# claussss/ubisoft-laforge-daft-exprt

Hardware: AMD Instinct MI355X
Metric: mel frames/sec (fwd+bwd) (higher is better)
Workload: dtype bf16; 1 GPU; C2: LJ-shaped training step, 48 utterances/GPU, L_max=120, T_max=896, 28180 valid frames/GPU/step; forward + loss (mel L1/L2, adversarial CE, post-mult, energy + pitch consistency) + backward + fused Adam step (global-norm clip, LR schedule) + one-launch weight re-pack, dropout on; parallelism=dp1, launch=1 captured HIP graph(s) per step (one per backward phase) + eager optimiser

## Files before the change

### ubisoft_laforge_daft_exprt_amd/csrc/dx_ffpair.hip

```cpp
#include "dx_common.h"
#include <algorithm>

namespace {

template <int NJ> struct FP {
  static constexpr int NROW = NJ * 16;
  static constexpr int TOK = NROW - 2;
  static constexpr int HR = NROW + 2;
  static constexpr int IMG = 2 * HR * 128;
  static constexpr int XP = (HR * 16 + 511) / 512;
  static constexpr int RP = (HR + 31) / 32;
};
constexpr int FP_TOK = FP<8>::TOK;

struct FFPairArgs {
  const dx_h16* X; int ldx;
  const dx_h16* Wa; const dx_h16* Wb;
  const float* bias_a; const float* bias_b;
  const dx_h16* aux; int ld_aux;
  dx_h16* H; int ldh;
  float* Y; int ldy;
  int B, N, F;
  int accumulate;
  const int* lens; int skip_halo;
  const int* rows_exist;
  const float* ln_res; const float* ln_w; const float* ln_b; const float* film; int ld_film;
  float* ln_y; float* ln_mean; float* ln_rstd;
  unsigned long long seed_pre; unsigned thresh_pre; float inv_keep_pre; const unsigned long long* seed_offset;
  const dx_h16* q_w; const float* q_bias; dx_h16* q_out;
  const float* lnb_z; const float* lnb_mean; const float* lnb_rstd; const float* lnb_w; const float* lnb_b;
  dx_h16* lnb_dg; float* lnb_dw; float* lnb_db;
  const dx_h16* lnb_wt; dx_h16* lnb_datt;
  const float* lnp_dy; const float* lnp_z; const float* lnp_mean; const float* lnp_rstd; const float* lnp_w; const float* lnp_b;
  const float* lnp_film; int lnp_ld_film;
  dx_h16* lnp_dg; float* lnp_dw; float* lnp_db; float* lnp_dfilm; int lnp_ld_dfilm;
  unsigned long long lnp_seed; unsigned lnp_thresh; float lnp_inv_keep;
  unsigned* hmask;
  unsigned long long* stamps;
};

#ifdef DX_FFPAIR_STAMPS
#define FP_STAMP(K) { if (lane == 0 && wq == 0 && a.stamps) a.stamps[((size_t)blockIdx.x * 2 + role) * 16 + (K)] = __builtin_amdgcn_s_memtime(); }
#else
#define FP_STAMP(K) {}
#endif

__device__ __forceinline__ int fp_lds_off(int row, int slot) { return row * 128 + ((slot ^ (row & 7)) << 4); }

__device__ __forceinline__ uint2 fp_pack4(float a, float b, float c, float d) {
  bf16x4 h;
  h[0] = (dx_h16)a; h[1] = (dx_h16)b; h[2] = (dx_h16)c; h[3] = (dx_h16)d;
  return __builtin_bit_cast(uint2, h);
}

__device__ __forceinline__ int fp_opaque(int x) { asm volatile("" : "+v"(x)); return x; }

__device__ __forceinline__ int fp_wave_sum_i(int v) {
#pragma unroll
  for (int off = 32; off > 0; off >>= 1) v += __shfl_xor(v, off, 64);
  return v;
}

typedef short s16x2 __attribute__((ext_vector_type(2)));

#define FP_MMA(W, X, C) C = DX_MFMA_H16(__builtin_bit_cast(bf16x8, W), __builtin_bit_cast(bf16x8, X), C);
// ... 101 lines not shown
        if (a.lnp_w) *reinterpret_cast<f32x4*>(a.lnp_dg + ((size_t)b * a.N + n0 + row) * 128 + q * 8) = f32x4{0.f, 0.f, 0.f, 0.f};
        if (a.lnb_wt) *reinterpret_cast<f32x4*>(a.lnb_datt + ((size_t)b * a.N + n0 + row) * 128 + q * 8) = f32x4{0.f, 0.f, 0.f, 0.f};
      }
    if (a.lnp_w)
      for (int u = tid; u < rows * 32; u += 512) {
        const int row = u >> 5, q = u & 31;
        *reinterpret_cast<f32x4*>(a.Y + ((size_t)b * a.N + n0 + row) * a.ldy + q * 4) = f32x4{0.f, 0.f, 0.f, 0.f};
      }
    if (!a.accumulate)
      for (int u = tid; u < rows * 32; u += 512) {
        const int row = u >> 5, q = u & 31;
        *reinterpret_cast<f32x4*>(a.Y + ((size_t)b * a.N + n0 + row) * a.ldy + q * 4) = f32x4{0.f, 0.f, 0.f, 0.f};
        if (a.ln_w) *reinterpret_cast<f32x4*>(a.ln_y + ((size_t)b * a.N + n0 + row) * 128 + q * 4) = f32x4{0.f, 0.f, 0.f, 0.f};
      }
    if (a.q_w)
      for (int u = tid; u < rows * 48; u += 512) {
        const int row = u / 48, q = u - row * 48;
        *reinterpret_cast<f32x4*>(a.q_out + ((size_t)b * a.N + n0 + row) * 384 + q * 8) = f32x4{0.f, 0.f, 0.f, 0.f};
      }
    return;
  }

  const int NL = a.rows_exist ? a.rows_exist[b] : a.N;
  if (a.lnp_w) {
    const int q = tid & 15;
    const int len_b = a.lens ? a.lens[b] : a.N;
    float wv[8], bv[8], fg[8];
#pragma unroll
    for (int e = 0; e < 8; ++e) {
      wv[e] = a.lnp_w[q * 8 + e]; bv[e] = a.lnp_b[q * 8 + e];
      fg[e] = a.lnp_film ? a.lnp_film[(size_t)b * a.lnp_ld_film + q * 8 + e] : 1.f;
    }
    const unsigned long long seed = a.lnp_seed + (a.seed_offset ? *a.seed_offset : 0ull);
    float gw[8], gb[8], gfg[8], gfb[8];
#pragma unroll
    for (int e = 0; e < 8; ++e) gw[e] = gb[e] = gfg[e] = gfb[e] = 0.f;
    f32x4 dyv[RP][2], zv[RP][2];
    float muv[RP], rsv[RP];
#pragma unroll
    for (int it = 0; it < RP; ++it) {
      const int row = (tid >> 4) + it * 32, n = n0 - 2 + row;
      const bool valid = row < FP_HR && n >= 0 && n < len_b && n < NL;
      const size_t grow = (size_t)b * a.N + n;
#pragma unroll
      for (int hh = 0; hh < 2; ++hh) {
        dyv[it][hh] = valid ? *reinterpret_cast<const f32x4*>(a.lnp_dy + grow * 128 + q * 8 + hh * 4) : f32x4{0.f, 0.f, 0.f, 0.f};
        zv[it][hh] = valid ? *reinterpret_cast<const f32x4*>(a.lnp_z + grow * 128 + q * 8 + hh * 4) : f32x4{0.f, 0.f, 0.f, 0.f};
      }
      muv[it] = valid ? a.lnp_mean[grow] : 0.f;
      rsv[it] = valid ? a.lnp_rstd[grow] : 0.f;
    }
    FP_WLOAD(0, 0) FP_WLOAD(1, 1) FP_WLOAD(2, 2) FP_WLOAD(3, 3)
    if constexpr (RING == 6) { FP_WLOAD(4, 4) FP_WLOAD(5, 5) }
#pragma unroll
    for (int it = 0; it < RP; ++it) {
      const int row = (tid >> 4) + it * 32, n = n0 - 2 + row;
      const bool inb = row < FP_HR && n >= 0 && n < a.N;
      const bool owned = inb && row >= 2 && row < 2 + FP_TOK;
      const bool ownvalid = owned && n < len_b;
      const size_t grow = (size_t)b * a.N + n;
      float dz[8];
      float s1 = 0.f, s2 = 0.f, g[8], xh[8];
#pragma unroll
      for (int e = 0; e < 8; ++e) {
        const float z = zv[it][e >> 2][e & 3];
        float d = dyv[it][e >> 2][e & 3];
        xh[e] = (z - muv[it]) * rsv[it];
        const float ln = xh[e] * wv[e] + bv[e];
        if (ownvalid) { gfg[e] += d * ln; gfb[e] += d; }
        d *= fg[e];
        if (ownvalid) { gw[e] += d * xh[e]; gb[e] += d; }
        g[e] = d * wv[e];
        s1 += g[e]; s2 += g[e] * xh[e];
      }
#pragma unroll
      for (int off = 1; off < 16; off <<= 1) { s1 += __shfl_xor(s1, off, 64); s2 += __shfl_xor(s2, off, 64); }
      s1 *= (1.0f / 128); s2 *= (1.0f / 128);
#pragma unroll
      for (int e = 0; e < 8; ++e) dz[e] = rsv[it] * (g[e] - s1 - xh[e] * s2);
      if (owned) {
        if (dzs && row - 2 < DZ_ROWS) {
          *reinterpret_cast<f32x4*>(dzs + (row - 2) * 128 + q * 8) = f32x4{dz[0], dz[1], dz[2], dz[3]};
          *reinterpret_cast<f32x4*>(dzs + (row - 2) * 128 + q * 8 + 4) = f32x4{dz[4], dz[5], dz[6], dz[7]};
        } else {
          *reinterpret_cast<f32x4*>(a.Y + grow * a.ldy + q * 8) = f32x4{dz[0], dz[1], dz[2], dz[3]};
          *reinterpret_cast<f32x4*>(a.Y + grow * a.ldy + q * 8 + 4) = f32x4{dz[4], dz[5], dz[6], dz[7]};
        }
      }
      if (a.lnp_thresh) {
        float f[8];
        dx_dropout_scale4(seed, (unsigned long long)grow * 128 + q * 8, a.lnp_thresh, a.lnp_inv_keep, f);
        dx_dropout_scale4(seed, (unsigned long long)grow * 128 + q * 8 + 4, a.lnp_thresh, a.lnp_inv_keep, f + 4);
#pragma unroll
        for (int e = 0; e < 8; ++e) dz[e] *= f[e];
      }
      bf16x8 h8;
#pragma unroll
      for (int e = 0; e < 8; ++e) h8[e] = (dx_h16)dz[e];
      const f32x4 hv = __builtin_bit_cast(f32x4, h8);
      if (owned) *reinterpret_cast<f32x4*>(a.lnp_dg + grow * 128 + q * 8) = hv;
      if (row < FP_HR) *reinterpret_cast<f32x4*>(Xs + (q >> 3) * (FP_HR * 128) + fp_lds_off(row, q & 7)) = hv;
    }
#pragma unroll
    for (int e = 0; e < 8; ++e) {
#pragma unroll
      for (int off = 16; off < 64; off <<= 1) {
        gw[e] += __shfl_xor(gw[e], off, 64); gb[e] += __shfl_xor(gb[e], off, 64);
        gfg[e] += __shfl_xor(gfg[e], off, 64); gfb[e] += __shfl_xor(gfb[e], off, 64);
      }
    }
    float* const red = reinterpret_cast<float*>(Hs0);
    if (lane < 16) {
#pragma unroll
      for (int e = 0; e < 8; ++e) {
        red[(wave * 4 + 0) * 128 + q * 8 + e] = gw[e]; red[(wave * 4 + 1) * 128 + q * 8 + e] = gb[e];
        red[(wave * 4 + 2) * 128 + q * 8 + e] = gfg[e]; red[(wave * 4 + 3) * 128 + q * 8 + e] = gfb[e];
      }
    }
    __syncthreads();
    {
      const int quant = tid >> 7, c = tid & 127;
      float t = 0.f;
#pragma unroll
      for (int w8 = 0; w8 < 8; ++w8) t += red[(w8 * 4 + quant) * 128 + c];
      if (t != 0.f) {
        if (quant == 0) atomicAdd(&a.lnp_dw[c], t);
        else if (quant == 1) atomicAdd(&a.lnp_db[c], t);
        else if (a.lnp_dfilm) atomicAdd(&a.lnp_dfilm[(size_t)b * a.lnp_ld_dfilm + (quant == 3 ? 128 : 0) + c], t);
      }
    }
    __syncthreads();
    if (tid < 64) {
      const int img = tid >> 5, rr = NROW + ((tid >> 4) & 1), qq = tid & 15;
      *reinterpret_cast<f32x4*>((img ? Hs1 : Hs0) + (qq >> 3) * (FP_HR * 128) + fp_lds_off(rr, qq & 7)) = f32x4{0.f, 0.f, 0.f, 0.f};
    }
  } else
  {
    f32x4 xr[XP];
#pragma unroll
    for (int it = 0; it < XP; ++it) {
      const int u = tid + it * 512;
      const int row = u >> 4, q = u & 15;
      const int n = n0 - 2 + row;
      f32x4 v = f32x4{0.f, 0.f, 0.f, 0.f};
      if (u < FP_HR * 16 && n >= 0 && n < NL) v = *reinterpret_cast<const f32x4*>(a.X + ((size_t)b * a.N + n) * a.ldx + q * 8);
      xr[it] = v;
    }
    FP_WLOAD(0, 0) FP_WLOAD(1, 1) FP_WLOAD(2, 2) FP_WLOAD(3, 3)
    if constexpr (RING == 6) { FP_WLOAD(4, 4) FP_WLOAD(5, 5) }
    if (tid < 64) {
      const int img = tid >> 5, rr = NROW + ((tid >> 4) & 1), q = tid & 15;
      *reinterpret_cast<f32x4*>((img ? Hs1 : Hs0) + (q >> 3) * (FP_HR * 128) + fp_lds_off(rr, q & 7)) = f32x4{0.f, 0.f, 0.f, 0.f};
    }
#pragma unroll
    for (int it = 0; it < XP; ++it) {
      const int u = tid + it * 512;
      const int row = u >> 4, q = u & 15;
      if (u < FP_HR * 16) *reinterpret_cast<f32x4*>(Xs + (q >> 3) * (FP_HR * 128) + fp_lds_off(row, q & 7)) = xr[it];
    }
  }
  __syncthreads();
  FP_STAMP(2)

  int foff[3][2];
#pragma unroll
  for (int t = 0; t < 3; ++t)
#pragma unroll
    for (int hh = 0; hh < 2; ++hh) foff[t][hh] = fp_lds_off(r + t, hh * 4 + g);
  const int len_cols = min(FP_TOK, a.N - n0);
  const int h_rows = a.H ? len_cols : 0;

#define FP_CO_RD(K, IMGC)                                                                                            \
  {                                                                                                                  \
    const int u_ = fp_opaque(tid) + NROW * 8 + (K) * 256;        \
    const int row_ = u_ >> 4, q_ = u_ & 15;                                                                          \
    cpv = *reinterpret_cast<const f32x4*>((IMGC) + (q_ >> 3) * (FP_HR * 128) + fp_lds_off(min(row_, NROW - 1) + 1, q_ & 7)); \
  }
#define FP_CO_ST(K, F0C)                                                                                             \
  {                                                                                                                  \
    const int u_ = fp_opaque(tid) + NROW * 8 + (K) * 256;                                                            \
    const int row_ = u_ >> 4, q_ = u_ & 15;                                                                          \
    if (row_ < h_rows) *reinterpret_cast<f32x4*>(a.H + ((size_t)b * a.N + n0 + row_) * a.ldh + (F0C) + q_ * 8) = cpv; \
  }
#define FP_COPY_OUT_CONS(IMGC, F0C)                                                                                  \
  {                                                                                                                  \
    f32x4 cv_[NJ / 2];                                                                                               \
    const int t_ = fp_opaque(tid) - 256;                        \
    _Pragma("unroll") for (int k = 0; k < NJ / 2; ++k) {                                                                  \
      const int u_ = t_ + k * 256;                                                                                   \
      cv_[k] = *reinterpret_cast<const f32x4*>((IMGC) + ((u_ & 15) >> 3) * (FP_HR * 128) + fp_lds_off((u_ >> 4) + 1, u_ & 7)); \
    }                                                                                                                \
    _Pragma("unroll") for (int k = 0; k < NJ / 2; ++k) {                                                             \
      const int u_ = t_ + k * 256;                                                                                   \
      const int row_ = u_ >> 4, q_ = u_ & 15;                                                                        \
      if (row_ < h_rows) *reinterpret_cast<f32x4*>(a.H + ((size_t)b * a.N + n0 + row_) * a.ldh + (F0C) + q_ * 8) = cv_[k]; \
    }                                                                                                                \
  }

#define FP_RD8(DST, IMG, S)                                                                                          \
  {                                                                                                                  \
    const unsigned char* const bp_ = (IMG) + (((S) & 3) >> 1) * (FP_HR * 128) + foff[((S) >> 2) % 3][(S) & 1];       \
    _Pragma("unroll") for (int j = 0; j < NJ; ++j) DST[j] = *reinterpret_cast<const float4*>(bp_ + j * 2048);        \
  }
#define FP_STEP(CUR, NXT, IMG, GS0, S, AUXPF, FRESH, CO, IMGC, F0C)                                                  \
  {                                                                                                                  \
    if ((S) + 1 < 12) FP_RD8(NXT, IMG, (S) + 1)                                                                      \
    if ((CO) && (S) < NJ && ((S) & 1) == 0) FP_CO_RD((S) >> 1, IMGC)                                                 \
    __builtin_amdgcn_sched_barrier(0);                                                                               \
    const f32x4 w0 = wr[(S) % RING][0], w1 = wr[(S) % RING][1];                                                      \
    if ((FRESH) && (S) == 0) {                                   \
      _Pragma("unroll") for (int j = 0; j < NJ; ++j) { acc[0][j] = bv0; FP_MMA(w0, CUR[j], acc[0][j]) }              \
      _Pragma("unroll") for (int j = 0; j < NJ; ++j) { acc[1][j] = bv1; FP_MMA(w1, CUR[j], acc[1][j]) }              \
    } else {                                                                                                         \
      _Pragma("unroll") for (int j = 0; j < NJ; ++j) { FP_MMA(w0, CUR[j], acc[0][j]) }                               \
      _Pragma("unroll") for (int j = 0; j < NJ; ++j) { FP_MMA(w1, CUR[j], acc[1][j]) }                               \
    }                                                                                                                \
    FP_WLOAD((S) % RING, (GS0) + (S) + RING)                                                                         \
    if ((CO) && (S) < NJ && ((S) & 1) == 1) FP_CO_ST((S) >> 1, F0C)                                                  \
    if ((S) == 8) { AUXPF }                                                                                          \
    __builtin_amdgcn_sched_barrier(0);                                                                               \
  }
#define FP_SLICE_STEPS(IMG, GS0, AUXPF, FR, CO, IMGC, F0C)                                                           \
  {                                                                                                                  \
    float4 xa[NJ], xb[NJ];                                                                                           \
    f32x4 cpv;                                                                                                       \
    FP_RD8(xa, IMG, 0)                                                                                               \
    FP_STEP(xa, xb, IMG, GS0, 0, AUXPF, FR, CO, IMGC, F0C) FP_STEP(xb, xa, IMG, GS0, 1, AUXPF, FR, CO, IMGC, F0C)    \
    FP_STEP(xa, xb, IMG, GS0, 2, AUXPF, FR, CO, IMGC, F0C) FP_STEP(xb, xa, IMG, GS0, 3, AUXPF, FR, CO, IMGC, F0C)    \
    FP_STEP(xa, xb, IMG, GS0, 4, AUXPF, FR, CO, IMGC, F0C) FP_STEP(xb, xa, IMG, GS0, 5, AUXPF, FR, CO, IMGC, F0C)    \
    FP_STEP(xa, xb, IMG, GS0, 6, AUXPF, FR, CO, IMGC, F0C) FP_STEP(xb, xa, IMG, GS0, 7, AUXPF, FR, CO, IMGC, F0C)    \
    FP_STEP(xa, xb, IMG, GS0, 8, AUXPF, FR, CO, IMGC, F0C) FP_STEP(xb, xa, IMG, GS0, 9, AUXPF, FR, CO, IMGC, F0C)    \
    FP_STEP(xa, xb, IMG, GS0, 10, AUXPF, FR, CO, IMGC, F0C) FP_STEP(xb, xa, IMG, GS0, 11, AUXPF, FR, CO, IMGC, F0C)  \
  }

  unsigned char* const stage = smem;
  if (role == 0) {
    f32x4 acc[2][NJ];
    const bool edge = n0 == 0 || n0 + FP_TOK >= NL;
    const int tile_lin = b * tiles_n + n0 / FP_TOK;
#define FP_PRODUCE(F_, COFLAG)                                                                                       \
    {                                                                                                                \
      const int f0 = (F_) << 7;                                                                                      \
                                   \
      const f32x4 bv0 = a.bias_a ? *reinterpret_cast<const f32x4*>(a.bias_a + f0 + 32 * wq + 4 * g) : f32x4{0.f, 0.f, 0.f, 0.f};      \
      const f32x4 bv1 = a.bias_a ? *reinterpret_cast<const f32x4*>(a.bias_a + f0 + 32 * wq + 16 + 4 * g) : f32x4{0.f, 0.f, 0.f, 0.f}; \
      bf16x4 av[2][MASK ? 1 : NJ];                                                                                   \
      unsigned mw[2] = {0u, 0u};                                                                                     \
      FP_SLICE_STEPS(Xs, (F_) * 12,                                                                                  \
        if constexpr (AUX) {                                                                                         \
          if constexpr (MASK) {                                                                                      \
            const unsigned* mp_ = a.hmask + ((((size_t)tile_lin * nslices + (f0 >> 7)) * 4 + wq) * 2) * 64 + fp_opaque(lane); \
            mw[0] = mp_[0]; mw[1] = mp_[64];                                                                         \
          } else {                                                                                                   \
          const int r2_ = fp_opaque(r);                                                                              \
          const int g2_ = fp_opaque(g);                                                                              \
          _Pragma("unroll") for (int i = 0; i < 2; ++i)                                                              \
            _Pragma("unroll") for (int j = 0; j < NJ; ++j) {                                                         \
              const int n = min(max(n0 - 1 + 16 * j + r2_, 0), a.N - 1);                                             \
              av[i][j] = *reinterpret_cast<const bf16x4*>(a.aux + ((size_t)b * a.N + n) * a.ld_aux + f0 + 32 * wq + 16 * i + 4 * g2_); \
            }                                                                                                        \
          }                                                                                                          \
        }, true, COFLAG, ((((F_) - 1) & 1) ? Hs1 : Hs0), ((F_) - 1) * 128)                                           \
      unsigned char* const out = ((F_) & 1) ? Hs1 : Hs0;                                                             \
      const int r_ = fp_opaque(r);                                                                                   \
      const int g_ = fp_opaque(g);                                                                                   \
      _Pragma("unroll") for (int i = 0; i < 2; ++i) {                                                                \
        const int c = 32 * wq + 16 * i + 4 * g_;                                                                     \
        unsigned char* const orow = out + (c >> 6) * (FP_HR * 128) + fp_lds_off(r_, (c & 63) >> 3) + ((g_ & 1) << 3); \
        unsigned sw_ = 0u;                                                  \
        const unsigned mwi_ = mw[i];                                                                                 \
        _Pragma("unroll") for (int j = 0; j < NJ; ++j) {                                                             \
          f32x4 v = acc[i][j];                                                                                       \
          if constexpr (AUX) {                                                                                       \
            if constexpr (MASK) {                                                                                    \
               \
              _Pragma("unroll") for (int e = 0; e < 4; ++e) {                                                        \
                const float ve_ = v[e];                                                                              \
                const unsigned ke_ = __float_as_uint(ve_) & (unsigned)__builtin_amdgcn_sbfe((int)mwi_, NJ * 4 - 1 - (j * 4 + e), 1); \
                v[e] = __uint_as_float(ke_);                                                                         \
              }                                                                                                      \
            } else {                                                                                                 \
              _Pragma("unroll") for (int e = 0; e < 4; ++e) if (!((float)av[i][j][e] > 0.f)) v[e] = 0.f;             \
            }                                                                                                        \
          }                                                                                                          \
          if (edge) { const int n = n0 - 1 + 16 * j + r_; if (n < 0 || n >= NL) v = f32x4{0.f, 0.f, 0.f, 0.f}; }    \
          if constexpr (RELU) {                                                                                      \
             \
            if (a.hmask) {                                                                                           \
              _Pragma("unroll") for (int e = 0; e < 4; ++e) {                                                        \
                const float ve_ = v[e];                                                                              \
                sw_ = __builtin_amdgcn_alignbit(sw_, __float_as_uint(ve_) - 1u, 31);                                 \
              }                                                                                                      \
            }                                                                                                        \
          }                                                                                                          \
          uint2 pk = fp_pack4(v[0], v[1], v[2], v[3]);                                                               \
          if constexpr (RELU) {                                                                                      \
             \
            pk.x = __builtin_bit_cast(unsigned, __builtin_elementwise_max(__builtin_bit_cast(s16x2, pk.x), s16x2{0, 0})); \
            pk.y = __builtin_bit_cast(unsigned, __builtin_elementwise_max(__builtin_bit_cast(s16x2, pk.y), s16x2{0, 0})); \
          }                                                                                                          \
          *reinterpret_cast<uint2*>(orow + j * 2048) = pk;                                                           \
        }                                                                                                            \
        if constexpr (RELU) {                                        \
          if (a.hmask) a.hmask[((((size_t)tile_lin * nslices + (f0 >> 7)) * 4 + wq) * 2 + i) * 64 + fp_opaque(lane)] = ~sw_; \
        }                                                                                                            \
      }                                                                                                              \
    }
    FP_PRODUCE(0, false)
    __syncthreads();
    FP_STAMP(3)
    for (int it = 1; it < nslices; ++it) {
      if (it == 4) FP_STAMP(12)
      FP_PRODUCE(it, true)
      if (it == 4) FP_STAMP(14)
      __syncthreads();
      FP_STAMP(3 + it)
    }
    {
      const unsigned char* const imgc = ((nslices - 1) & 1) ? Hs1 : Hs0;
      f32x4 cpv;
#pragma unroll
      for (int k = 0; k < NJ / 2; ++k) { FP_CO_RD(k, imgc) FP_CO_ST(k, (nslices - 1) << 7) }
    }
    __syncthreads();
    FP_STAMP(3 + nslices)
#undef FP_PRODUCE
  } else {
    f32x4 acc[2][NJ];
    const f32x4 bv0 = f32x4{0.f, 0.f, 0.f, 0.f}, bv1 = bv0;
#pragma unroll
    for (int i = 0; i < 2; ++i)
#pragma unroll
      for (int j = 0; j < NJ; ++j) acc[i][j] = f32x4{0.f, 0.f, 0.f, 0.f};
    __syncthreads();
    FP_STAMP(3)
    for (int it = 1; it <= nslices; ++it) {
      if (it == 4) FP_STAMP(12)
      const int f = it - 1;
      const unsigned char* const img = (f & 1) ? Hs1 : Hs0;
      FP_COPY_OUT_CONS(img, f << 7)
      FP_SLICE_STEPS(img, f * 12, , false, false, img, 0)
      if (it == 4) FP_STAMP(13)
      __syncthreads();
      FP_STAMP(3 + it)
    }
#pragma unroll
    for (int i = 0; i < 2; ++i) {
      const int co = 32 * wq + 16 * i + 4 * g;
      const f32x4 bv = a.bias_b ? *reinterpret_cast<const f32x4*>(a.bias_b + co) : f32x4{0.f, 0.f, 0.f, 0.f};
#pragma unroll
      for (int j = 0; j < NJ; ++j) {
        const int q = 16 * j + r;
        *reinterpret_cast<f32x4*>(stage + q * 512 + (((co >> 2) ^ (q & 15)) << 4)) = acc[i][j] + bv;
      }
    }
  }
#undef FP_SLICE_STEPS
#undef FP_STEP
#undef FP_RD8
#undef FP_COPY_OUT_CONS
#undef FP_CO_RD
#undef FP_CO_ST

  __syncthreads();
  if (a.ln_w) {
    const int s = tid & 31;
    const f32x4 wv = *reinterpret_cast<const f32x4*>(a.ln_w + s * 4), bv = *reinterpret_cast<const f32x4*>(a.ln_b + s * 4);
    f32x4 fg = f32x4{1.f, 1.f, 1.f, 1.f}, fb = f32x4{0.f, 0.f, 0.f, 0.f};
    if (a.film) {
      fg = *reinterpret_cast<const f32x4*>(a.film + (size_t)b * a.ld_film + s * 4);
      fb = *reinterpret_cast<const f32x4*>(a.film + (size_t)b * a.ld_film + 128 + s * 4);
    }
    const int len_b = a.lens ? a.lens[b] : a.N;
    const unsigned long long seed = a.seed_pre + (a.seed_offset ? *a.seed_offset : 0ull);
    bf16x8 qa[3][4];
    if (a.q_w) {
#pragma unroll
      for (int i = 0; i < 3; ++i)
#pragma unroll
        for (int ks = 0; ks < 4; ++ks) qa[i][ks] = *reinterpret_cast<const bf16x8*>(a.q_w + (size_t)((wave * 3 + i) * 4 + ks) * 512 + lane * 8);
    }
    f32x4 resv[NJ];
#pragma unroll
    for (int k = 0; k < NJ; ++k) {
      const int row = (tid >> 5) + k * 16, n = n0 + row;
      resv[k] = (row < len_cols && n < len_b) ? *reinterpret_cast<const f32x4*>(a.ln_res + ((size_t)b * a.N + n) * 128 + s * 4) : f32x4{0.f, 0.f, 0.f, 0.f};
    }
#pragma unroll
    for (int k = 0; k < NJ; ++k) {
      const int row = (tid >> 5) + k * 16, n = n0 + row;
      const bool inb = row < len_cols, valid = inb && n < len_b;
      const size_t grow = (size_t)b * a.N + n;
      f32x4 z = f32x4{0.f, 0.f, 0.f, 0.f};
      if (valid) {
        z = *reinterpret_cast<const f32x4*>(stage + row * 512 + ((s ^ (row & 15)) << 4));
        if (a.thresh_pre) {
          float f[4];
          dx_dropout_scale4(seed, (unsigned long long)grow * 128 + s * 4, a.thresh_pre, a.inv_keep_pre, f);
          z[0] *= f[0]; z[1] *= f[1]; z[2] *= f[2]; z[3] *= f[3];
        }
        z += resv[k];
      }
      if (inb) *reinterpret_cast<f32x4*>(a.Y + grow * a.ldy + s * 4) = z;
      float sum = (z[0] + z[1]) + (z[2] + z[3]);
#pragma unroll
      for (int off = 1; off < 32; off <<= 1) sum += __shfl_xor(sum, off, 64);
      const float mu = sum * (1.0f / 128);
      const f32x4 d = z - mu;
      float q = (d[0] * d[0] + d[1] * d[1]) + (d[2] * d[2] + d[3] * d[3]);
#pragma unroll
// ... 21 lines not shown
        bf16x8 xb[4];
#pragma unroll
        for (int ks = 0; ks < 4; ++ks) xb[ks] = *reinterpret_cast<const bf16x8*>(stage + row * 512 + (((ks * 4 + g) ^ (row & 15)) << 4));
        f32x4 acc[3];
#pragma unroll
        for (int i = 0; i < 3; ++i) acc[i] = qb[i];
#pragma unroll
        for (int ks = 0; ks < 4; ++ks)
#pragma unroll
          for (int i = 0; i < 3; ++i) acc[i] = DX_MFMA_H16(qa[i][ks], xb[ks], acc[i]);
        if (row < len_cols) {
          dx_h16* const orow = a.q_out + ((size_t)b * a.N + n0 + row) * 384 + wave * 48 + g * 4;
#pragma unroll
          for (int i = 0; i < 3; ++i) {
            bf16x4 o4;
            o4[0] = (dx_h16)acc[i][0]; o4[1] = (dx_h16)acc[i][1]; o4[2] = (dx_h16)acc[i][2]; o4[3] = (dx_h16)acc[i][3];
            *reinterpret_cast<bf16x4*>(orow + i * 16) = o4;
          }
        }
      }
    }
  } else if (a.lnb_w) {
    const int s = tid & 31;
    const f32x4 wv = *reinterpret_cast<const f32x4*>(a.lnb_w + s * 4), bv = *reinterpret_cast<const f32x4*>(a.lnb_b + s * 4);
    (void)bv;
    const int len_b = a.lens ? a.lens[b] : a.N;
    const unsigned long long seed = a.seed_pre + (a.seed_offset ? *a.seed_offset : 0ull);
    f32x4 oldv[NJ], zv[NJ];
    float muv[NJ], rsv[NJ];
#pragma unroll
    for (int k = 0; k < NJ; ++k) {
      const int row = (tid >> 5) + k * 16, n = n0 + row;
      const bool valid = row < len_cols && n < len_b;
      const size_t grow = (size_t)b * a.N + n;
      if (dzs && row < DZ_ROWS) oldv[k] = valid ? *reinterpret_cast<const f32x4*>(dzs + row * 128 + s * 4) : f32x4{0.f, 0.f, 0.f, 0.f};
      else oldv[k] = valid ? *reinterpret_cast<const f32x4*>(a.Y + grow * a.ldy + s * 4) : f32x4{0.f, 0.f, 0.f, 0.f};
      zv[k] = valid ? *reinterpret_cast<const f32x4*>(a.lnb_z + grow * 128 + s * 4) : f32x4{0.f, 0.f, 0.f, 0.f};
      muv[k] = valid ? a.lnb_mean[grow] : 0.f;
      rsv[k] = valid ? a.lnb_rstd[grow] : 0.f;
    }
    f32x4 gw = f32x4{0.f, 0.f, 0.f, 0.f}, gb = gw;
#pragma unroll
    for (int k = 0; k < NJ; ++k) {
      const int row = (tid >> 5) + k * 16, n = n0 + row;
      const bool inb = row < len_cols, valid = inb && n < len_b;
      const size_t grow = (size_t)b * a.N + n;
      f32x4 d = f32x4{0.f, 0.f, 0.f, 0.f};
      if (valid) d = *reinterpret_cast<const f32x4*>(stage + row * 512 + ((s ^ (row & 15)) << 4)) + oldv[k];
      const f32x4 xh = (zv[k] - muv[k]) * rsv[k];
      gw += d * xh; gb += d;
      const f32x4 g = d * wv;
      float s1 = (g[0] + g[1]) + (g[2] + g[3]);
      const f32x4 gx = g * xh;
      float s2 = (gx[0] + gx[1]) + (gx[2] + gx[3]);
#pragma unroll
      for (int off = 1; off < 32; off <<= 1) { s1 += __shfl_xor(s1, off, 64); s2 += __shfl_xor(s2, off, 64); }
      s1 *= (1.0f / 128); s2 *= (1.0f / 128);
      f32x4 dz = (g - s1 - xh * s2) * rsv[k];
      if (!inb) continue;
      *reinterpret_cast<f32x4*>(a.Y + grow * a.ldy + s * 4) = dz;
      if (a.thresh_pre) {
        float f[4];
        dx_dropout_scale4(seed, (unsigned long long)grow * 128 + s * 4, a.thresh_pre, a.inv_keep_pre, f);
        dz[0] *= f[0]; dz[1] *= f[1]; dz[2] *= f[2]; dz[3] *= f[3];
      }
      bf16x4 h4;
      h4[0] = (dx_h16)dz[0]; h4[1] = (dx_h16)dz[1]; h4[2] = (dx_h16)dz[2]; h4[3] = (dx_h16)dz[3];
      *reinterpret_cast<bf16x4*>(a.lnb_dg + grow * 128 + s * 4) = h4;
      if (a.lnb_wt) *reinterpret_cast<bf16x4*>(stage + row * 512 + (((s >> 1) ^ (row & 15)) << 4) + ((s & 1) << 3)) = h4;
    }
    if (a.lnb_wt) {
#pragma unroll
      for (int k = 0; k < NJ; ++k) {
        const int row = (tid >> 5) + k * 16;
        if (row >= len_cols) *reinterpret_cast<uint2*>(stage + row * 512 + (((s >> 1) ^ (row & 15)) << 4) + ((s & 1) << 3)) = make_uint2(0u, 0u);
      }
    }
    float* const red = reinterpret_cast<float*>(smem + NROW * 512);
    *reinterpret_cast<f32x4*>(red + (tid >> 5) * 128 + s * 4) = gw;
    *reinterpret_cast<f32x4*>(red + 2048 + (tid >> 5) * 128 + s * 4) = gb;
    __syncthreads();
    if (tid < 256) {
      const float* src = red + (tid >> 7) * 2048 + (tid & 127);
      float t = 0.f;
#pragma unroll
      for (int q = 0; q < 16; ++q) t += src[q * 128];
      if (t != 0.f) atomicAdd((tid >> 7) ? &a.lnb_db[tid & 127] : &a.lnb_dw[tid & 127], t);
    }
    if (a.lnb_wt) {
      constexpr int CB = NJ;
      const int rb = wave % NJ, cb0 = (wave / NJ) * CB;
      const int row = rb * 16 + r;
      bf16x8 xb[4];
#pragma unroll
      for (int ks = 0; ks < 4; ++ks) xb[ks] = *reinterpret_cast<const bf16x8*>(stage + row * 512 + (((ks * 4 + g) ^ (row & 15)) << 4));
      f32x4 acc[CB];
#pragma unroll
      for (int i = 0; i < CB; ++i) acc[i] = f32x4{0.f, 0.f, 0.f, 0.f};
#pragma unroll
      for (int ks = 0; ks < 4; ++ks) {
        bf16x8 wa[CB];
#pragma unroll
        for (int i = 0; i < CB; ++i) wa[i] = *reinterpret_cast<const bf16x8*>(a.lnb_wt + (size_t)((cb0 + i) * 4 + ks) * 512 + lane * 8);
#pragma unroll
        for (int i = 0; i < CB; ++i) acc[i] = DX_MFMA_H16(wa[i], xb[ks], acc[i]);
      }
      if (row < len_cols) {
        dx_h16* const orow = a.lnb_datt + ((size_t)b * a.N + n0 + row) * 128 + cb0 * 16 + g * 4;
#pragma unroll
        for (int i = 0; i < CB; ++i) {
          bf16x4 o4;
          o4[0] = (dx_h16)acc[i][0]; o4[1] = (dx_h16)acc[i][1]; o4[2] = (dx_h16)acc[i][2]; o4[3] = (dx_h16)acc[i][3];
          *reinterpret_cast<bf16x4*>(orow + i * 16) = o4;
        }
      }
    }
  } else {
    f32x4 old[NJ];
    if (a.accumulate) {
#pragma unroll
      for (int k = 0; k < NJ; ++k) {
        const int u = tid + k * 512;
        const int row = min(u >> 5, len_cols - 1), s = u & 31;
        old[k] = *reinterpret_cast<const f32x4*>(a.Y + ((size_t)b * a.N + n0 + row) * a.ldy + s * 4);
      }
    }
#pragma unroll
    for (int k = 0; k < NJ; ++k) {
      const int u = tid + k * 512;
// ... 167 lines not shown
```

Before: 4.804 million valid mel frames/s.

## Split LN-backward prologue across roles and prefetch epilogue operands before final sync

For the aux NJ=8 fused FF-pair kernel, the LN-backward prologue rows are split. Role 0 finishes its part early and starts the first producer slice in two halves, while role 1 processes the remaining halo rows and does the parameter-gradient reduction, removing the block-wide barrier before the GEMM. Epilogue operands (LN weights, film, residual/z rows, mean/rstd, q_w fragments, lnb_wt weights) are now fetched into registers before the last barrier so their latency overlaps compute. This raises register pressure and adds complex role-dependent synchronisation, which risks spills, occupancy loss or barrier mismatch.

```diff
diff --git a/ubisoft_laforge_daft_exprt_amd/csrc/dx_ffpair.hip b/ubisoft_laforge_daft_exprt_amd/csrc/dx_ffpair.hip
--- a/ubisoft_laforge_daft_exprt_amd/csrc/dx_ffpair.hip
+++ b/ubisoft_laforge_daft_exprt_amd/csrc/dx_ffpair.hip
@@ -40,7 +40,7 @@
 };
 
 #ifdef DX_FFPAIR_STAMPS
-#define FP_STAMP(K) { if (lane == 0 && wq == 0 && a.stamps) a.stamps[((size_t)blockIdx.x * 2 + role) * 16 + (K)] = __builtin_amdgcn_s_memtime(); }
+#define FP_STAMP(K) { if (lane == 0 && wq == 0 && a.stamps) a.stamps[((size_t)blockIdx.x * 2 + role) * 24 + (K)] = __builtin_amdgcn_s_memtime(); }
 #else
 #define FP_STAMP(K) {}
 #endif
@@ -188,6 +188,10 @@
   }
 
   const int NL = a.rows_exist ? a.rows_exist[b] : a.N;
+  constexpr bool SPLIT = AUX && NJ == 8;
+  constexpr int PA = SPLIT ? 3 : RP;
+  constexpr int PB = SPLIT ? (FP_HR - PA * 32 + 15) / 16 : 0;
+  const bool split0 = SPLIT && a.lnp_w != nullptr;
   if (a.lnp_w) {
     const int q = tid & 15;
     const int len_b = a.lens ? a.lens[b] : a.N;
@@ -201,26 +205,20 @@
     float gw[8], gb[8], gfg[8], gfb[8];
 #pragma unroll
     for (int e = 0; e < 8; ++e) gw[e] = gb[e] = gfg[e] = gfb[e] = 0.f;
-    f32x4 dyv[RP][2], zv[RP][2];
-    float muv[RP], rsv[RP];
-#pragma unroll
-    for (int it = 0; it < RP; ++it) {
-      const int row = (tid >> 4) + it * 32, n = n0 - 2 + row;
+    auto row_load = [&](int row, f32x4 (&dy)[2], f32x4 (&z)[2], float& mu, float& rs) {
+      const int n = n0 - 2 + row;
       const bool valid = row < FP_HR && n >= 0 && n < len_b && n < NL;
       const size_t grow = (size_t)b * a.N + n;
 #pragma unroll
       for (int hh = 0; hh < 2; ++hh) {
-        dyv[it][hh] = valid ? *reinterpret_cast<const f32x4*>(a.lnp_dy + grow * 128 + q * 8 + hh * 4) : f32x4{0.f, 0.f, 0.f, 0.f};
-        zv[it][hh] = valid ? *reinterpret_cast<const f32x4*>(a.lnp_z + grow * 128 + q * 8 + hh * 4) : f32x4{0.f, 0.f, 0.f, 0.f};
-      }
-      muv[it] = valid ? a.lnp_mean[grow] : 0.f;
-      rsv[it] = valid ? a.lnp_rstd[grow] : 0.f;
-    }
-    FP_WLOAD(0, 0) FP_WLOAD(1, 1) FP_WLOAD(2, 2) FP_WLOAD(3, 3)
-    if constexpr (RING == 6) { FP_WLOAD(4, 4) FP_WLOAD(5, 5) }
-#pragma unroll
-    for (int it = 0; it < RP; ++it) {
-      const int row = (tid >> 4) + it * 32, n = n0 - 2 + row;
+        dy[hh] = valid ? *reinterpret_cast<const f32x4*>(a.lnp_dy + grow * 128 + q * 8 + hh * 4) : f32x4{0.f, 0.f, 0.f, 0.f};
+        z[hh] = valid ? *reinterpret_cast<const f32x4*>(a.lnp_z + grow * 128 + q * 8 + hh * 4) : f32x4{0.f, 0.f, 0.f, 0.f};
+      }
+      mu = valid ? a.lnp_mean[grow] : 0.f;
+      rs = valid ? a.lnp_rstd[grow] : 0.f;
+    };
+    auto row_pass = [&](int row, const f32x4 (&dy)[2], const f32x4 (&zz)[2], float mu, float rs) {
+      const int n = n0 - 2 + row;
       const bool inb = row < FP_HR && n >= 0 && n < a.N;
       const bool owned = inb && row >= 2 && row < 2 + FP_TOK;
       const bool ownvalid = owned && n < len_b;
@@ -229,9 +227,9 @@
       float s1 = 0.f, s2 = 0.f, g[8], xh[8];
 #pragma unroll
       for (int e = 0; e < 8; ++e) {
-        const float z = zv[it][e >> 2][e & 3];
-        float d = dyv[it][e >> 2][e & 3];
-        xh[e] = (z - muv[it]) * rsv[it];
+        const float z = zz[e >> 2][e & 3];
+        float d = dy[e >> 2][e & 3];
+        xh[e] = (z - mu) * rs;
         const float ln = xh[e] * wv[e] + bv[e];
         if (ownvalid) { gfg[e] += d * ln; gfb[e] += d; }
         d *= fg[e];
@@ -243,7 +241,7 @@
       for (int off = 1; off < 16; off <<= 1) { s1 += __shfl_xor(s1, off, 64); s2 += __shfl_xor(s2, off, 64); }
       s1 *= (1.0f / 128); s2 *= (1.0f / 128);
 #pragma unroll
-      for (int e = 0; e < 8; ++e) dz[e] = rsv[it] * (g[e] - s1 - xh[e] * s2);
+      for (int e = 0; e < 8; ++e) dz[e] = rs * (g[e] - s1 - xh[e] * s2);
       if (owned) {
         if (dzs && row - 2 < DZ_ROWS) {
           *reinterpret_cast<f32x4*>(dzs + (row - 2) * 128 + q * 8) = f32x4{dz[0], dz[1], dz[2], dz[3]};
@@ -266,39 +264,102 @@
       const f32x4 hv = __builtin_bit_cast(f32x4, h8);
       if (owned) *reinterpret_cast<f32x4*>(a.lnp_dg + grow * 128 + q * 8) = hv;
       if (row < FP_HR) *reinterpret_cast<f32x4*>(Xs + (q >> 3) * (FP_HR * 128) + fp_lds_off(row, q & 7)) = hv;
-    }
-#pragma unroll
-    for (int e = 0; e < 8; ++e) {
-#pragma unroll
-      for (int off = 16; off < 64; off <<= 1) {
-        gw[e] += __shfl_xor(gw[e], off, 64); gb[e] += __shfl_xor(gb[e], off, 64);
-        gfg[e] += __shfl_xor(gfg[e], off, 64); gfb[e] += __shfl_xor(gfb[e], off, 64);
-      }
-    }
-    float* const red = reinterpret_cast<float*>(Hs0);
-    if (lane < 16) {
+    };
+    auto wave_fold = [&]() {
 #pragma unroll
       for (int e = 0; e < 8; ++e) {
-        red[(wave * 4 + 0) * 128 + q * 8 + e] = gw[e]; red[(wave * 4 + 1) * 128 + q * 8 + e] = gb[e];
-        red[(wave * 4 + 2) * 128 + q * 8 + e] = gfg[e]; red[(wave * 4 + 3) * 128 + q * 8 + e] = gfb[e];
-      }
-    }
-    __syncthreads();
-    {
-      const int quant = tid >> 7, c = tid & 127;
-      float t = 0.f;
-#pragma unroll
-      for (int w8 = 0; w8 < 8; ++w8) t += red[(w8 * 4 + quant) * 128 + c];
+#pragma unroll
+        for (int off = 16; off < 64; off <<= 1) {
+          gw[e] += __shfl_xor(gw[e], off, 64); gb[e] += __shfl_xor(gb[e], off, 64);
+          gfg[e] += __shfl_xor(gfg[e], off, 64); gfb[e] += __shfl_xor(gfb[e], off, 64);
+        }
+      }
+    };
+    auto red_atomic = [&](int quant, int c, float t) {
       if (t != 0.f) {
         if (quant == 0) atomicAdd(&a.lnp_dw[c], t);
         else if (quant == 1) atomicAdd(&a.lnp_db[c], t);
         else if (a.lnp_dfilm) atomicAdd(&a.lnp_dfilm[(size_t)b * a.lnp_ld_dfilm + (quant == 3 ? 128 : 0) + c], t);
       }
-    }
-    __syncthreads();
-    if (tid < 64) {
-      const int img = tid >> 5, rr = NROW + ((tid >> 4) & 1), qq = tid & 15;
-      *reinterpret_cast<f32x4*>((img ? Hs1 : Hs0) + (qq >> 3) * (FP_HR * 128) + fp_lds_off(rr, qq & 7)) = f32x4{0.f, 0.f, 0.f, 0.f};
+    };
+    {
+      f32x4 dyv[PA][2], zv[PA][2];
+      float muv[PA], rsv[PA];
+#pragma unroll
+      for (int it = 0; it < PA; ++it) row_load((tid >> 4) + it * 32, dyv[it], zv[it], muv[it], rsv[it]);
+      FP_WLOAD(0, 0) FP_WLOAD(1, 1) FP_WLOAD(2, 2) FP_WLOAD(3, 3)
+      if constexpr (RING == 6) { FP_WLOAD(4, 4) FP_WLOAD(5, 5) }
+#pragma unroll
+      for (int it = 0; it < PA; ++it) row_pass((tid >> 4) + it * 32, dyv[it], zv[it], muv[it], rsv[it]);
+    }
+    if constexpr (SPLIT) {
+      if (tid < 64) {
+        const int img = tid >> 5, rr = NROW + ((tid >> 4) & 1), qq = tid & 15;
+        *reinterpret_cast<f32x4*>((img ? Hs1 : Hs0) + (qq >> 3) * (FP_HR * 128) + fp_lds_off(rr, qq & 7)) = f32x4{0.f, 0.f, 0.f, 0.f};
+      }
+      float* const red = reinterpret_cast<float*>(Hs1);
+      if (role == 0) {
+        wave_fold();
+        if (lane < 16) {
+#pragma unroll
+          for (int e = 0; e < 8; ++e) {
+            red[(wq * 4 + 0) * 128 + q * 8 + e] = gw[e]; red[(wq * 4 + 1) * 128 + q * 8 + e] = gb[e];
+            red[(wq * 4 + 2) * 128 + q * 8 + e] = gfg[e]; red[(wq * 4 + 3) * 128 + q * 8 + e] = gfb[e];
+          }
+        }
+        __syncthreads();
+      } else {
+        f32x4 dyv[PB][2], zv[PB][2];
+        float muv[PB], rsv[PB];
+        const int row0 = PA * 32 + ((tid - 256) >> 4);
+#pragma unroll
+        for (int it = 0; it < PB; ++it) row_load(row0 + it * 16, dyv[it], zv[it], muv[it], rsv[it]);
+        __syncthreads();
+        FP_STAMP(2)
+#pragma unroll
+        for (int it = 0; it < PB; ++it) row_pass(row0 + it * 16, dyv[it], zv[it], muv[it], rsv[it]);
+        wave_fold();
+        if (lane < 16) {
+#pragma unroll
+          for (int e = 0; e < 8; ++e) {
+            red[(wq * 4 + 0) * 128 + q * 8 + e] += gw[e]; red[(wq * 4 + 1) * 128 + q * 8 + e] += gb[e];
+            red[(wq * 4 + 2) * 128 + q * 8 + e] += gfg[e]; red[(wq * 4 + 3) * 128 + q * 8 + e] += gfb[e];
+          }
+        }
+        __syncthreads();
+        FP_STAMP(16)
+#pragma unroll
+        for (int hh = 0; hh < 2; ++hh) {
+          const int u = tid - 256 + hh * 256, quant = u >> 7, c = u & 127;
+          float t = 0.f;
+#pragma unroll
+          for (int w4 = 0; w4 < 4; ++w4) t += red[(w4 * 4 + quant) * 128 + c];
+          red_atomic(quant, c, t);
+        }
+      }
+    } else {
+      wave_fold();
+      float* const red = reinterpret_cast<float*>(Hs0);
+      if (lane < 16) {
+#pragma unroll
+        for (int e = 0; e < 8; ++e) {
+          red[(wave * 4 + 0) * 128 + q * 8 + e] = gw[e]; red[(wave * 4 + 1) * 128 + q * 8 + e] = gb[e];
+          red[(wave * 4 + 2) * 128 + q * 8 + e] = gfg[e]; red[(wave * 4 + 3) * 128 + q * 8 + e] = gfb[e];
+        }
+      }
+      __syncthreads();
+      {
+        const int quant = tid >> 7, c = tid & 127;
+        float t = 0.f;
+#pragma unroll
+        for (int w8 = 0; w8 < 8; ++w8) t += red[(w8 * 4 + quant) * 128 + c];
+        red_atomic(quant, c, t);
+      }
+      __syncthreads();
+      if (tid < 64) {
+        const int img = tid >> 5, rr = NROW + ((tid >> 4) & 1), qq = tid & 15;
+        *reinterpret_cast<f32x4*>((img ? Hs1 : Hs0) + (qq >> 3) * (FP_HR * 128) + fp_lds_off(rr, qq & 7)) = f32x4{0.f, 0.f, 0.f, 0.f};
+      }
     }
   } else
   {
@@ -325,8 +386,8 @@
       if (u < FP_HR * 16) *reinterpret_cast<f32x4*>(Xs + (q >> 3) * (FP_HR * 128) + fp_lds_off(row, q & 7)) = xr[it];
     }
   }
-  __syncthreads();
-  FP_STAMP(2)
+  if (!split0) __syncthreads();
+  if (!(split0 && role == 1)) FP_STAMP(2)
 
   int foff[3][2];
 #pragma unroll
@@ -363,48 +424,105 @@
     }                                                                                                                \
   }
 
-#define FP_RD8(DST, IMG, S)                                                                                          \
+#define FP_RD8(DST, IMG, S, JLO, JHI)                                                                                \
   {                                                                                                                  \
     const unsigned char* const bp_ = (IMG) + (((S) & 3) >> 1) * (FP_HR * 128) + foff[((S) >> 2) % 3][(S) & 1];       \
-    _Pragma("unroll") for (int j = 0; j < NJ; ++j) DST[j] = *reinterpret_cast<const float4*>(bp_ + j * 2048);        \
-  }
-#define FP_STEP(CUR, NXT, IMG, GS0, S, AUXPF, FRESH, CO, IMGC, F0C)                                                  \
+    _Pragma("unroll") for (int j = (JLO); j < (JHI); ++j) DST[j] = *reinterpret_cast<const float4*>(bp_ + j * 2048); \
+  }
+#define FP_STEP(CUR, NXT, IMG, GS0, S, AUXPF, FRESH, CO, IMGC, F0C, JLO, JHI, WRAP)                                                \
   {                                                                                                                  \
-    if ((S) + 1 < 12) FP_RD8(NXT, IMG, (S) + 1)                                                                      \
+    if ((S) + 1 < 12) FP_RD8(NXT, IMG, (S) + 1, JLO, JHI)                                                            \
     if ((CO) && (S) < NJ && ((S) & 1) == 0) FP_CO_RD((S) >> 1, IMGC)                                                 \
     __builtin_amdgcn_sched_barrier(0);                                                                               \
     const f32x4 w0 = wr[(S) % RING][0], w1 = wr[(S) % RING][1];                                                      \
     if ((FRESH) && (S) == 0) {                                   \
-      _Pragma("unroll") for (int j = 0; j < NJ; ++j) { acc[0][j] = bv0; FP_MMA(w0, CUR[j], acc[0][j]) }              \
-      _Pragma("unroll") for (int j = 0; j < NJ; ++j) { acc[1][j] = bv1; FP_MMA(w1, CUR[j], acc[1][j]) }              \
+      _Pragma("unroll") for (int j = (JLO); j < (JHI); ++j) { acc[0][j] = bv0; FP_MMA(w0, CUR[j], acc[0][j]) }       \
+      _Pragma("unroll") for (int j = (JLO); j < (JHI); ++j) { acc[1][j] = bv1; FP_MMA(w1, CUR[j], acc[1][j]) }       \
     } else {                                                                                                         \
-      _Pragma("unroll") for (int j = 0; j < NJ; ++j) { FP_MMA(w0, CUR[j], acc[0][j]) }                               \
-      _Pragma("unroll") for (int j = 0; j < NJ; ++j) { FP_MMA(w1, CUR[j], acc[1][j]) }                               \
+      _Pragma("unroll") for (int j = (JLO); j < (JHI); ++j) { FP_MMA(w0, CUR[j], acc[0][j]) }                        \
+      _Pragma("unroll") for (int j = (JLO); j < (JHI); ++j) { FP_MMA(w1, CUR[j], acc[1][j]) }                        \
     }                                                                                                                \
-    FP_WLOAD((S) % RING, (GS0) + (S) + RING)                                                                         \
+     \
+    FP_WLOAD((S) % RING, (GS0) + ((WRAP) ? ((S) + RING) % 12 : (S) + RING))                                          \
     if ((CO) && (S) < NJ && ((S) & 1) == 1) FP_CO_ST((S) >> 1, F0C)                                                  \
     if ((S) == 8) { AUXPF }                                                                                          \
     __builtin_amdgcn_sched_barrier(0);                                                                               \
   }
-#define FP_SLICE_STEPS(IMG, GS0, AUXPF, FR, CO, IMGC, F0C)                                                           \
+#define FP_SLICE_STEPS(IMG, GS0, AUXPF, FR, CO, IMGC, F0C, JLO, JHI, WRAP)                                          \
   {                                                                                                                  \
     float4 xa[NJ], xb[NJ];                                                                                           \
     f32x4 cpv;                                                                                                       \
-    FP_RD8(xa, IMG, 0)                                                                                               \
-    FP_STEP(xa, xb, IMG, GS0, 0, AUXPF, FR, CO, IMGC, F0C) FP_STEP(xb, xa, IMG, GS0, 1, AUXPF, FR, CO, IMGC, F0C)    \
-    FP_STEP(xa, xb, IMG, GS0, 2, AUXPF, FR, CO, IMGC, F0C) FP_STEP(xb, xa, IMG, GS0, 3, AUXPF, FR, CO, IMGC, F0C)    \
-    FP_STEP(xa, xb, IMG, GS0, 4, AUXPF, FR, CO, IMGC, F0C) FP_STEP(xb, xa, IMG, GS0, 5, AUXPF, FR, CO, IMGC, F0C)    \
-    FP_STEP(xa, xb, IMG, GS0, 6, AUXPF, FR, CO, IMGC, F0C) FP_STEP(xb, xa, IMG, GS0, 7, AUXPF, FR, CO, IMGC, F0C)    \
-    FP_STEP(xa, xb, IMG, GS0, 8, AUXPF, FR, CO, IMGC, F0C) FP_STEP(xb, xa, IMG, GS0, 9, AUXPF, FR, CO, IMGC, F0C)    \
-    FP_STEP(xa, xb, IMG, GS0, 10, AUXPF, FR, CO, IMGC, F0C) FP_STEP(xb, xa, IMG, GS0, 11, AUXPF, FR, CO, IMGC, F0C)  \
+    FP_RD8(xa, IMG, 0, JLO, JHI)                                                                                     \
+    FP_STEP(xa, xb, IMG, GS0, 0, AUXPF, FR, CO, IMGC, F0C, JLO, JHI, WRAP) FP_STEP(xb, xa, IMG, GS0, 1, AUXPF, FR, CO, IMGC, F0C, JLO, JHI, WRAP)   \
+    FP_STEP(xa, xb, IMG, GS0, 2, AUXPF, FR, CO, IMGC, F0C, JLO, JHI, WRAP) FP_STEP(xb, xa, IMG, GS0, 3, AUXPF, FR, CO, IMGC, F0C, JLO, JHI, WRAP)   \
+    FP_STEP(xa, xb, IMG, GS0, 4, AUXPF, FR, CO, IMGC, F0C, JLO, JHI, WRAP) FP_STEP(xb, xa, IMG, GS0, 5, AUXPF, FR, CO, IMGC, F0C, JLO, JHI, WRAP)   \
+    FP_STEP(xa, xb, IMG, GS0, 6, AUXPF, FR, CO, IMGC, F0C, JLO, JHI, WRAP) FP_STEP(xb, xa, IMG, GS0, 7, AUXPF, FR, CO, IMGC, F0C, JLO, JHI, WRAP)   \
+    FP_STEP(xa, xb, IMG, GS0, 8, AUXPF, FR, CO, IMGC, F0C, JLO, JHI, WRAP) FP_STEP(xb, xa, IMG, GS0, 9, AUXPF, FR, CO, IMGC, F0C, JLO, JHI, WRAP)   \
+    FP_STEP(xa, xb, IMG, GS0, 10, AUXPF, FR, CO, IMGC, F0C, JLO, JHI, WRAP) FP_STEP(xb, xa, IMG, GS0, 11, AUXPF, FR, CO, IMGC, F0C, JLO, JHI, WRAP) \
   }
 
   unsigned char* const stage = smem;
+  f32x4 ev[NJ], e_wv, e_bv, e_fg, e_fb;
+  float emu[NJ], ers[NJ];
+  bf16x8 e_qa[3][4];
+#define FP_EPI_FETCH                                                                                                 \
+  {                                                                                                                  \
+    const int s_ = fp_opaque(tid) & 31, t5_ = fp_opaque(tid) >> 5;                                                   \
+    if constexpr (AUX) {                                                                                             \
+      if (a.lnb_w) {                                                                                                 \
+        const int len_b_ = a.lens ? a.lens[b] : a.N;                                                                 \
+        e_wv = *reinterpret_cast<const f32x4*>(a.lnb_w + s_ * 4);                                                    \
+        _Pragma("unroll") for (int k = 0; k < NJ; ++k) {                                                             \
+          const int row = t5_ + k * 16, n = n0 + row;                                                                \
+          const bool valid = row < len_cols && n < len_b_;                                                           \
+          const size_t grow = (size_t)b * a.N + n;                                                                   \
+          ev[k] = valid ? *reinterpret_cast<const f32x4*>(a.lnb_z + grow * 128 + s_ * 4) : f32x4{0.f, 0.f, 0.f, 0.f}; \
+          emu[k] = valid ? a.lnb_mean[grow] : 0.f;                                                                   \
+          ers[k] = valid ? a.lnb_rstd[grow] : 0.f;                                                                   \
+        }                                                                                                            \
+      }                                                                                                              \
+    } else {                                                                                                         \
+      if (a.ln_w) {                                                                                                  \
+        const int len_b_ = a.lens ? a.lens[b] : a.N;                                                                 \
+        e_wv = *reinterpret_cast<const f32x4*>(a.ln_w + s_ * 4); e_bv = *reinterpret_cast<const f32x4*>(a.ln_b + s_ * 4); \
+        e_fg = f32x4{1.f, 1.f, 1.f, 1.f}; e_fb = f32x4{0.f, 0.f, 0.f, 0.f};                                          \
+        if (a.film) {                                                                                                \
+          e_fg = *reinterpret_cast<const f32x4*>(a.film + (size_t)b * a.ld_film + s_ * 4);                           \
+          e_fb = *reinterpret_cast<const f32x4*>(a.film + (size_t)b * a.ld_film + 128 + s_ * 4);                     \
+        }                                                                                                            \
+        if (a.q_w) {                                                    \
+          _Pragma("unroll") for (int i = 0; i < 3; ++i)                                                              \
+            _Pragma("unroll") for (int ks = 0; ks < 4; ++ks)                                                         \
+              e_qa[i][ks] = *reinterpret_cast<const bf16x8*>(a.q_w + (size_t)((wave * 3 + i) * 4 + ks) * 512 + fp_opaque(lane) * 8); \
+        }                                                                                                            \
+        _Pragma("unroll") for (int k = 0; k < NJ; ++k) {                                                             \
+          const int row = t5_ + k * 16, n = n0 + row;                                                                \
+          ev[k] = (row < len_cols && n < len_b_) ? *reinterpret_cast<const f32x4*>(a.ln_res + ((size_t)b * a.N + n) * 128 + s_ * 4) \
+                                                 : f32x4{0.f, 0.f, 0.f, 0.f};                                        \
+        }                                                                                                            \
+      }                                                                                                              \
+    }                                                                                                                \
+  }
   if (role == 0) {
     f32x4 acc[2][NJ];
     const bool edge = n0 == 0 || n0 + FP_TOK >= NL;
     const int tile_lin = b * tiles_n + n0 / FP_TOK;
-#define FP_PRODUCE(F_, COFLAG)                                                                                       \
+#define FP_AUX_PREFETCH                                                                                              \
+    if constexpr (AUX) {                                                                                             \
+      if constexpr (MASK) {                                                                                          \
+        const unsigned* mp_ = a.hmask + ((((size_t)tile_lin * nslices + (f0 >> 7)) * 4 + wq) * 2) * 64 + fp_opaque(lane);\
+        mw[0] = mp_[0]; mw[1] = mp_[64];                                                                             \
+      } else {                                                                                                       \
+      const int r2_ = fp_opaque(r);                                                                                  \
+      const int g2_ = fp_opaque(g);                                                                                  \
+      _Pragma("unroll") for (int i = 0; i < 2; ++i)                                                                  \
+        _Pragma("unroll") for (int j = 0; j < NJ; ++j) {                                                             \
+          const int n = min(max(n0 - 1 + 16 * j + r2_, 0), a.N - 1);                                                 \
+          av[i][j] = *reinterpret_cast<const bf16x4*>(a.aux + ((size_t)b * a.N + n) * a.ld_aux + f0 + 32 * wq + 16 * i + 4 * g2_);\
+        }                                                                                                            \
+      }                                                                                                              \
+    }
+#define FP_PRODUCE(F_, COFLAG, SPLIT0)                                                                                       \
     {                                                                                                                \
       const int f0 = (F_) << 7;                                                                                      \
                                    \
@@ -412,21 +530,16 @@
       const f32x4 bv1 = a.bias_a ? *reinterpret_cast<const f32x4*>(a.bias_a + f0 + 32 * wq + 16 + 4 * g) : f32x4{0.f, 0.f, 0.f, 0.f}; \
       bf16x4 av[2][MASK ? 1 : NJ];                                                                                   \
       unsigned mw[2] = {0u, 0u};                                                                                     \
-      FP_SLICE_STEPS(Xs, (F_) * 12,                                                                                  \
-        if constexpr (AUX) {                                                                                         \
-          if constexpr (MASK) {                                                                                      \
-            const unsigned* mp_ = a.hmask + ((((size_t)tile_lin * nslices + (f0 >> 7)) * 4 + wq) * 2) * 64 + fp_opaque(lane); \
-            mw[0] = mp_[0]; mw[1] = mp_[64];                                                                         \
-          } else {                                                                                                   \
-          const int r2_ = fp_opaque(r);                                                                              \
-          const int g2_ = fp_opaque(g);                                                                              \
-          _Pragma("unroll") for (int i = 0; i < 2; ++i)                                                              \
-            _Pragma("unroll") for (int j = 0; j < NJ; ++j) {                                                         \
-              const int n = min(max(n0 - 1 + 16 * j + r2_, 0), a.N - 1);                                             \
-              av[i][j] = *reinterpret_cast<const bf16x4*>(a.aux + ((size_t)b * a.N + n) * a.ld_aux + f0 + 32 * wq + 16 * i + 4 * g2_); \
-            }                                                                                                        \
-          }                                                                                                          \
-        }, true, COFLAG, ((((F_) - 1) & 1) ? Hs1 : Hs0), ((F_) - 1) * 128)                                           \
+      if (SPLIT0) {                                                                                                  \
+         \
+                    \
+        FP_SLICE_STEPS(Xs, 0, , true, false, Hs0, 0, 0, NJ / 2, true)                                                \
+        __syncthreads();                                                                                             \
+        FP_STAMP(16)                                                                                                 \
+        FP_SLICE_STEPS(Xs, 0, FP_AUX_PREFETCH, true, false, Hs0, 0, NJ / 2, NJ, false)                               \
+      } else {                                                                                                       \
+        FP_SLICE_STEPS(Xs, (F_) * 12, FP_AUX_PREFETCH, true, COFLAG, ((((F_) - 1) & 1) ? Hs1 : Hs0), ((F_) - 1) * 128, 0, NJ, false) \
+      }                                                                                                              \
       unsigned char* const out = ((F_) & 1) ? Hs1 : Hs0;                                                             \
       const int r_ = fp_opaque(r);                                                                                   \
       const int g_ = fp_opaque(g);                                                                                   \
@@ -472,16 +585,18 @@
         }                                                                                                            \
       }                                                                                                              \
     }
-    FP_PRODUCE(0, false)
+    FP_PRODUCE(0, false, split0)
     __syncthreads();
     FP_STAMP(3)
     for (int it = 1; it < nslices; ++it) {
       if (it == 4) FP_STAMP(12)
-      FP_PRODUCE(it, true)
+      FP_PRODUCE(it, true, false)
       if (it == 4) FP_STAMP(14)
       __syncthreads();
       FP_STAMP(3 + it)
     }
+    FP_EPI_FETCH
+    FP_STAMP(17)
     {
       const unsigned char* const imgc = ((nslices - 1) & 1) ? Hs1 : Hs0;
       f32x4 cpv;
@@ -491,6 +606,7 @@
     __syncthreads();
     FP_STAMP(3 + nslices)
 #undef FP_PRODUCE
+#undef FP_AUX_PREFETCH
   } else {
     f32x4 acc[2][NJ];
     const f32x4 bv0 = f32x4{0.f, 0.f, 0.f, 0.f}, bv1 = bv0;
@@ -505,11 +621,13 @@
       const int f = it - 1;
       const unsigned char* const img = (f & 1) ? Hs1 : Hs0;
       FP_COPY_OUT_CONS(img, f << 7)
-      FP_SLICE_STEPS(img, f * 12, , false, false, img, 0)
+      FP_SLICE_STEPS(img, f * 12, , false, false, img, 0, 0, NJ, false)
       if (it == 4) FP_STAMP(13)
       __syncthreads();
       FP_STAMP(3 + it)
     }
+    FP_EPI_FETCH
+    FP_STAMP(17)
 #pragma unroll
     for (int i = 0; i < 2; ++i) {
       const int co = 32 * wq + 16 * i + 4 * g;
@@ -521,6 +639,7 @@
       }
     }
   }
+#undef FP_EPI_FETCH
 #undef FP_SLICE_STEPS
 #undef FP_STEP
 #undef FP_RD8
@@ -531,27 +650,11 @@
   __syncthreads();
   if (a.ln_w) {
     const int s = tid & 31;
-    const f32x4 wv = *reinterpret_cast<const f32x4*>(a.ln_w + s * 4), bv = *reinterpret_cast<const f32x4*>(a.ln_b + s * 4);
-    f32x4 fg = f32x4{1.f, 1.f, 1.f, 1.f}, fb = f32x4{0.f, 0.f, 0.f, 0.f};
-    if (a.film) {
-      fg = *reinterpret_cast<const f32x4*>(a.film + (size_t)b * a.ld_film + s * 4);
-      fb = *reinterpret_cast<const f32x4*>(a.film + (size_t)b * a.ld_film + 128 + s * 4);
-    }
+    const f32x4 wv = e_wv, bv = e_bv, fg = e_fg, fb = e_fb;
     const int len_b = a.lens ? a.lens[b] : a.N;
     const unsigned long long seed = a.seed_pre + (a.seed_offset ? *a.seed_offset : 0ull);
-    bf16x8 qa[3][4];
-    if (a.q_w) {
-#pragma unroll
-      for (int i = 0; i < 3; ++i)
-#pragma unroll
-        for (int ks = 0; ks < 4; ++ks) qa[i][ks] = *reinterpret_cast<const bf16x8*>(a.q_w + (size_t)((wave * 3 + i) * 4 + ks) * 512 + lane * 8);
-    }
-    f32x4 resv[NJ];
-#pragma unroll
-    for (int k = 0; k < NJ; ++k) {
-      const int row = (tid >> 5) + k * 16, n = n0 + row;
-      resv[k] = (row < len_cols && n < len_b) ? *reinterpret_cast<const f32x4*>(a.ln_res + ((size_t)b * a.N + n) * 128 + s * 4) : f32x4{0.f, 0.f, 0.f, 0.f};
-    }
+    auto& qa = e_qa;
+    auto& resv = ev;
 #pragma unroll
     for (int k = 0; k < NJ; ++k) {
       const int row = (tid >> 5) + k * 16, n = n0 + row;
@@ -619,12 +722,11 @@
     }
   } else if (a.lnb_w) {
     const int s = tid & 31;
-    const f32x4 wv = *reinterpret_cast<const f32x4*>(a.lnb_w + s * 4), bv = *reinterpret_cast<const f32x4*>(a.lnb_b + s * 4);
-    (void)bv;
+    const f32x4 wv = e_wv;
     const int len_b = a.lens ? a.lens[b] : a.N;
     const unsigned long long seed = a.seed_pre + (a.seed_offset ? *a.seed_offset : 0ull);
-    f32x4 oldv[NJ], zv[NJ];
-    float muv[NJ], rsv[NJ];
+    f32x4 oldv[NJ];
+    auto& zv = ev; auto& muv = emu; auto& rsv = ers;
 #pragma unroll
     for (int k = 0; k < NJ; ++k) {
       const int row = (tid >> 5) + k * 16, n = n0 + row;
@@ -632,9 +734,6 @@
       const size_t grow = (size_t)b * a.N + n;
       if (dzs && row < DZ_ROWS) oldv[k] = valid ? *reinterpret_cast<const f32x4*>(dzs + row * 128 + s * 4) : f32x4{0.f, 0.f, 0.f, 0.f};
       else oldv[k] = valid ? *reinterpret_cast<const f32x4*>(a.Y + grow * a.ldy + s * 4) : f32x4{0.f, 0.f, 0.f, 0.f};
-      zv[k] = valid ? *reinterpret_cast<const f32x4*>(a.lnb_z + grow * 128 + s * 4) : f32x4{0.f, 0.f, 0.f, 0.f};
-      muv[k] = valid ? a.lnb_mean[grow] : 0.f;
-      rsv[k] = valid ? a.lnb_rstd[grow] : 0.f;
     }
     f32x4 gw = f32x4{0.f, 0.f, 0.f, 0.f}, gb = gw;
 #pragma unroll
@@ -673,6 +772,15 @@
         if (row >= len_cols) *reinterpret_cast<uint2*>(stage + row * 512 + (((s >> 1) ^ (row & 15)) << 4) + ((s & 1) << 3)) = make_uint2(0u, 0u);
       }
     }
+    constexpr int CB = NJ;
+    const int rb = wave % NJ, cb0 = (wave / NJ) * CB;
+    bf16x8 wa[4][CB];
+    if (a.lnb_wt) {
+#pragma unroll
+      for (int ks = 0; ks < 4; ++ks)
+#pragma unroll
+        for (int i = 0; i < CB; ++i) wa[ks][i] = *reinterpret_cast<const bf16x8*>(a.lnb_wt + (size_t)((cb0 + i) * 4 + ks) * 512 + lane * 8);
+    }
     float* const red = reinterpret_cast<float*>(smem + NROW * 512);
     *reinterpret_cast<f32x4*>(red + (tid >> 5) * 128 + s * 4) = gw;
     *reinterpret_cast<f32x4*>(red + 2048 + (tid >> 5) * 128 + s * 4) = gb;
@@ -685,8 +793,6 @@
       if (t != 0.f) atomicAdd((tid >> 7) ? &a.lnb_db[tid & 127] : &a.lnb_dw[tid & 127], t);
     }
     if (a.lnb_wt) {
-      constexpr int CB = NJ;
-      const int rb = wave % NJ, cb0 = (wave / NJ) * CB;
       const int row = rb * 16 + r;
       bf16x8 xb[4];
 #pragma unroll
@@ -695,13 +801,9 @@
 #pragma unroll
       for (int i = 0; i < CB; ++i) acc[i] = f32x4{0.f, 0.f, 0.f, 0.f};
 #pragma unroll
-      for (int ks = 0; ks < 4; ++ks) {
-        bf16x8 wa[CB];
-#pragma unroll
-        for (int i = 0; i < CB; ++i) wa[i] = *reinterpret_cast<const bf16x8*>(a.lnb_wt + (size_t)((cb0 + i) * 4 + ks) * 512 + lane * 8);
-#pragma unroll
-        for (int i = 0; i < CB; ++i) acc[i] = DX_MFMA_H16(wa[i], xb[ks], acc[i]);
-      }
+      for (int ks = 0; ks < 4; ++ks)
+#pragma unroll
+        for (int i = 0; i < CB; ++i) acc[i] = DX_MFMA_H16(wa[ks][i], xb[ks], acc[i]);
       if (row < len_cols) {
         dx_h16* const orow = a.lnb_datt + ((size_t)b * a.N + n0 + row) * 128 + cb0 * 16 + g * 4;
 #pragma unroll
```

Measured after the change: 4.829 million valid mel frames/s, median of 4. Within noise of the previous version (+0.5%).
